# befelix/safe_learning

Measured on NVIDIA B200. Metric: grid-point Lyapunov checks/sec (2D pendulum, M=500 GP), higher is better.
Workload: dtype f64

## Files before the change

### safe_learning_b200/csrc/filter.cu

```cuda
#define SLB_EVAL_NOINLINE 1
#include "common.cuh"

#include <atomic>
#include <string.h>
#include <stdlib.h>

#include "gp_mean_staged.cuh"
#include "gp_args.h"

namespace {

#ifndef SLB_FT
#define SLB_FT 64
#endif
#ifndef SLB_MEAN_MINB
#define SLB_MEAN_MINB 7
#endif
constexpr int FT = SLB_FT;
constexpr int HR = SLB_HEAD_RANK;
constexpr int HT = 512;
constexpr int HEAD_CTAS = 148;
constexpr int64_t CHUNK = 1 << 22;
constexpr int64_t WS_HEAD = 64 + SLB_SPLIT_TICKET_BYTES + (int64_t)SLB_SPLIT_PARTIAL_BYTES;


struct filter_side { double dec0, thr, guard, coef[SLB_MAX_OUT], z[SLB_MAX_IN], dm[SLB_MAX_OUT]; };

struct filter_args {
    int64_t n;
    int64_t idx_begin;
    uint8_t* negative;
    double* values;
    int64_t* list_a;
    filter_side* side_a;
    int64_t* list_b;
    unsigned long long* counts;
    unsigned long long* stats;
    int chunk_rows;
    int max_outputs_per_factor;
    int head_factors_staged;
    int screened;
    int mean_off[SLB_MAX_OUT];
    int mean_doubles;
    int prefetch_factors;
    double* probe_mu;
    double* probe_dm;
};

SLB_DEV int decide(const filter_side& t, const double* shi, int d) {
    double ub = 0.0, lb = 0.0;
    for (int j = 0; j < d; ++j) {
        const double e = t.coef[j] * shi[j];
        ub += fmax(e, 0.0);
        lb += fmin(e, 0.0);
        if (!(e == e)) { ub = e; lb = e; break; }
    }
    const double slack = t.guard + 1e-6 * (fabs(ub) + fabs(lb));
    if (t.dec0 + ub + slack < t.thr) return 1;
    if (t.dec0 + lb - slack >= t.thr) return 0;
    return -1;
}

SLB_DEV long long list_append(bool take, unsigned long long* counter) {
    const unsigned ballot = __ballot_sync(0xffffffffu, take);
    if (ballot == 0) return -1;
    const int lane = threadIdx.x & 31;
    unsigned long long base = 0;
    if (lane == __ffs(ballot) - 1) base = atomicAdd(counter, (unsigned long long)__popc(ballot));
    base = __shfl_sync(0xffffffffu, base, __ffs(ballot) - 1);
    return take ? (long long)(base + __popc(ballot & ((1u << lane) - 1))) : -1;
}

SLB_DEV void count_stat(bool hit, unsigned long long* slot) {
    const unsigned ballot = __ballot_sync(0xffffffffu, hit);
    if (ballot != 0 && (threadIdx.x & 31) == 0) atomicAdd(slot, (unsigned long long)__popc(ballot));
}

SLB_DEV void mean_decision_terms(const slb_sweep& cfg, filter_side& t, double vx, const double* mu,
                                 const double* mean_err) {
    const int D = cfg.gp.num_outputs;
    double vm[1];
    eval_fn_small(cfg.lyapunov, mu, vm);
    t.dec0 = f64sub(vm[0], vx);
    double lvmu = 0.0;
    double lverr = 0.0;
    {
        double lv[SLB_MAX_OUT];
        int nl = 1;
        if (cfg.lipschitz_v.kind != SLB_FN_NONE) nl = eval_fn_small(cfg.lipschitz_v, mu, lv);
        else lv[0] = cfg.lv_const;
        for (int j = 0; j < SLB_MAX_OUT; ++j) {
            const double l = j < D ? (nl == 1 ? lv[0] : lv[j]) : 0.0;
            t.coef[j] = j < D ? l * cfg.gp.outputs[j].beta : 0.0;
            if (j < D) { lvmu += fabs(l * mu[j]); lverr += fabs(l) * mean_err[j]; }
        }
    }
    t.guard = 1e-6 * (fabs(vm[0]) + fabs(vx) + fabs(t.thr) + lvmu) + 4.0 * lverr + 1e-300;
}

SLB_DEV double screening_slack(const slb_sweep& cfg, const double* mu, const double* dm,
                               const double* shi) {
    constexpr int NS = 4;
    const int D = cfg.gp.num_outputs;
    const slb_function& V = cfg.lyapunov;
    const int n = V.in_dim;
    double m[NS], d[NS], bs[NS], P[NS][NS];
#pragma unroll
    for (int i = 0; i < NS; ++i) {
        m[i] = i < n ? mu[i] : 0.0;
        d[i] = i < n ? dm[i] : 0.0;
        bs[i] = i < D ? fabs(cfg.gp.outputs[i].beta) * shi[i] : 0.0;
#pragma unroll
        for (int j = 0; j < NS; ++j) P[i][j] = (i < n && j < n) ? __ldg(V.matrix + i * n + j) : 0.0;
// ... 12 lines not shown
    double dl = 0.0;
    const slb_function& L = cfg.lipschitz_v;
    if (L.kind == SLB_FN_LINEAR) {
        const double sc = (L.flags & SLB_FLAG_SCALE) ? fabs(L.out_scale) : 1.0;
        const int mi = L.in_dim, mo = L.out_dim;
        double row[NS];
#pragma unroll
        for (int o = 0; o < NS; ++o) {
            row[o] = 0.0;
#pragma unroll
            for (int i = 0; i < NS; ++i)
                if (o < mo && i < mi) row[o] += fabs(__ldg(L.matrix + o * mi + i)) * d[i];
        }
        if ((L.flags & SLB_FLAG_NORM1) || mo == 1) {
            dl = sc * (row[0] + row[1] + row[2] + row[3]) * (bs[0] + bs[1] + bs[2] + bs[3]);
        } else {
#pragma unroll
            for (int j = 0; j < NS; ++j) dl += sc * row[j] * bs[j];
        }
    }
    return 1.000001 * (dv + dl);
}

template <int DIN>
__global__ void __launch_bounds__(FT, SLB_MEAN_MINB)
filter_mean_kernel(const __grid_constant__ slb_sweep cfg, const filter_args a) {
    extern __shared__ __align__(16) unsigned char smem_raw[];
    pdl_launch_dependents();
    prefetch_descriptor_operands(cfg);
    mean_pipe P;
    double *tab512, *tab64;
    mean_pipe_setup(P, smem_raw, DIN, a.chunk_rows, a.max_outputs_per_factor, cfg.gp, &tab512, &tab64);
    uint64_t* bar = P.bar;
    if (threadIdx.x == 0) mean_pipe_init(P, tab512);
    mean_pipe_start<DIN>(cfg.gp, P);
    __syncthreads();

    const int64_t rel0 = (int64_t)blockIdx.x * FT + threadIdx.x;
    const bool valid = rel0 < a.n;
    const int64_t rel = valid ? rel0 : a.n - 1;
    const int d = cfg.grid.ndim;
    const int D = cfg.gp.num_outputs;

    filter_side t;
    grid_index_to_state(cfg.grid, a.idx_begin + rel, t.z);
    double vx;
    lyapunov_state_terms(cfg, t.z, a.idx_begin + rel, &vx, &t.thr);
    {
        double u[SLB_MAX_OUT];
        const int m = eval_fn_small(cfg.policy, t.z, u);
        for (int c = 0; c < m; ++c) t.z[d + c] = u[c];
    }
    bool sane = true;
#pragma unroll
    for (int c = 0; c < DIN; ++c) sane &= fabs(t.z[c]) < 1e100;

    slb_bulk::mbar_wait(bar + 2, 0);
    double mu[SLB_MAX_OUT];
    double mean_err[SLB_MAX_OUT];
    gp_mean_staged<DIN, true>(cfg.gp, t.z, mu, mean_err, tab512, tab64, P);

    mean_decision_terms(cfg, t, vx, mu, mean_err);

    double shi[SLB_MAX_OUT];
    for (int j = 0; j < D; ++j) {
        const slb_gp_factor& F = cfg.gp.factors[cfg.gp.outputs[j].factor];
        shi[j] = sqrt(F.kernel.num_prims > 0 ? kernel_expr_diag<DIN>(F.kernel, t.z) : F.variance);
    }
    const int outcome = sane ? decide(t, shi, D) : -1;
    const bool undecided = valid && outcome < 0;
    if (valid) {
        a.negative[rel] = outcome > 0 ? 1 : 0;
        if (a.values != nullptr) a.values[rel] = vx;
    }
    const long long slot = list_append(undecided, a.counts + 0);
    if (undecided) { a.list_a[slot] = rel; a.side_a[slot] = t; }
    if (a.stats != nullptr) {
        count_stat(valid && !undecided, a.stats + 0);
        count_stat(valid, a.stats + 3);
    }
}

template <int DIN>
__global__ void __launch_bounds__(FT, SLB_MEAN_MINB)
filter_mean32_kernel(const __grid_constant__ slb_sweep cfg, const filter_args a) {
    extern __shared__ __align__(16) unsigned char smem_raw[];
    __shared__ double s_cen[SLB_MAX_IN];
    pdl_launch_dependents();
    prefetch_descriptor_operands(cfg);
    constexpr int W32 = row32<DIN>::W;
    mean_pipe P;
    P.bar = reinterpret_cast<uint64_t*>(smem_raw);
    P.C = a.chunk_rows;
    P.xstride = P.C * (DIN + 1);
    P.gstride = P.C * a.max_outputs_per_factor;
    P.xbuf = reinterpret_cast<double*>(smem_raw + 32);
    P.gbuf = P.xbuf + 2 * P.xstride;
    P.t = 0;
    mean32_bufs B;
    B.red = P.gbuf + 2 * P.gstride;
    B.xf = reinterpret_cast<float*>(B.red + 8 * (FT / 32) + 8);
    B.g = B.xf + P.C * W32;
    if (threadIdx.x == 0) {
        slb_bulk::mbar_init(P.bar + 0, 1);
        slb_bulk::mbar_init(P.bar + 1, 1);
        slb_bulk::fence_barrier_init();
        slb_bulk::fence_proxy_async();
    }
    mean_pipe_start<DIN>(cfg.gp, P);

    const int64_t rel0 = (int64_t)blockIdx.x * FT + threadIdx.x;
    const bool valid = rel0 < a.n;
    const int64_t rel = valid ? rel0 : a.n - 1;
    const int d = cfg.grid.ndim;
    const int D = cfg.gp.num_outputs;

    filter_side t;
    grid_index_to_state(cfg.grid, a.idx_begin + rel, t.z);
    double vx;
    lyapunov_state_terms(cfg, t.z, a.idx_begin + rel, &vx, &t.thr);
    {
        double u[SLB_MAX_OUT];
        const int m = eval_fn_small(cfg.policy, t.z, u);
        for (int c = 0; c < m; ++c) t.z[d + c] = u[c];
    }
    bool sane = true;
#pragma unroll
    for (int c = 0; c < DIN; ++c) sane &= fabs(t.z[c]) < 1e100;
    if (threadIdx.x == FT / 2) {
#pragma unroll
        for (int c = 0; c < DIN; ++c) s_cen[c] = t.z[c];
    }
    __syncthreads();
    double zcen[DIN];
#pragma unroll
    for (int c = 0; c < DIN; ++c) zcen[c] = s_cen[c];

    double mu[SLB_MAX_OUT], dm[SLB_MAX_OUT];
    gp_mean32_staged<DIN>(cfg.gp, t.z, zcen, mu, dm, sane, P, B);
    if (a.probe_mu != nullptr && valid) {
        for (int o = 0; o < D; ++o) {
            a.probe_mu[rel * D + o] = mu[o];
            a.probe_dm[rel * D + o] = sane ? dm[o] : __longlong_as_double(0x7ff0000000000000ll);
        }
    }

    double zero[SLB_MAX_OUT];
    for (int j = 0; j < SLB_MAX_OUT; ++j) zero[j] = 0.0;
    mean_decision_terms(cfg, t, vx, mu, zero);
    double shi[SLB_MAX_OUT];
    for (int j = 0; j < D; ++j) shi[j] = sqrt(cfg.gp.factors[cfg.gp.outputs[j].factor].variance);
    t.guard += screening_slack(cfg, mu, dm, shi);
    const int outcome = sane ? decide(t, shi, D) : -1;
    const bool undecided = valid && outcome < 0;
    if (valid) {
        a.negative[rel] = outcome > 0 ? 1 : 0;
        if (a.values != nullptr) a.values[rel] = vx;
    }
    const long long slot = list_append(undecided, a.counts + 0);
    if (undecided) {
        filter_side* dst = a.side_a + slot;
        dst->dec0 = vx;
        dst->thr = t.thr;
#pragma unroll
        for (int c = 0; c < DIN; ++c) dst->z[c] = t.z[c];
        for (int j = 0; j < D; ++j) {
            dst->coef[j] = mu[j];
            dst->dm[j] = sane ? dm[j] : __longlong_as_double(0x7ff0000000000000ll);
        }
        a.list_a[slot] = rel;
    }
    if (a.stats != nullptr) {
        count_stat(valid && !undecided, a.stats + 0);
        count_stat(valid, a.stats + 3);
    }
}

constexpr int HW = HT / 32;
constexpr int HP = 8;
constexpr int HP_SHORT = 2;

template <int DIN, int NO>
SLB_DEV void head_mean_factor(const double* __restrict__ xf, int Mp, const double* zs, double zz, int r,
                              int L, const double* __restrict__ tab512, double* dot) {
    constexpr int W = DIN + 1;
    const double* __restrict__ gm = xf + (size_t)Mp * W;
    double d0[NO], d1[NO];
#pragma unroll
    for (int q = 0; q < NO; ++q) { d0[q] = 0.0; d1[q] = 0.0; }
    for (int j = r; j < Mp; j += 4 * L) {
        double arg[4];
#pragma unroll
        for (int u = 0; u < 4; ++u) {
            const int jc = min(j + L * u, Mp - 1);
            double row[W];
            load_row<W>(xf + jc * W, row);
            double acc = row[DIN] + zz;
#pragma unroll
            for (int c = 0; c < DIN; ++c) acc = fma(zs[c], row[c], acc);
            arg[u] = acc;
        }
#pragma unroll
        for (int u = 0; u < 4; ++u) {
            bool far;
            double k = exp_neg_fast(arg[u], tab512, far);
            k = (far || j + L * u >= Mp) ? 0.0 : k;
            const int jc = min(j + L * u, Mp - 1);
#pragma unroll
            for (int q = 0; q < NO; ++q) {
                if (u & 1) d1[q] = fma(k, gm[q * Mp + jc], d1[q]);
                else d0[q] = fma(k, gm[q * Mp + jc], d0[q]);
            }
        }
    }
#pragma unroll
    for (int q = 0; q < NO; ++q) {
        double v = d0[q] + d1[q];
        for (int off = L >> 1; off > 0; off >>= 1) v += __shfl_xor_sync(0xffffffffu, v, off);
        dot[q] = v;
    }
}

template <int DIN>
SLB_DEV void head_round_means(const slb_sweep& cfg, const filter_args& a, const int* slots, int nneed,
                              int64_t grp0, int64_t count, const double* mbuf, const double* tab512,
                              double* mu_s, double* merr_s) {
    const int nf = cfg.gp.num_factors, D = cfg.gp.num_outputs;
    const int L = nneed <= 16 ? 32 : nneed <= 32 ? 16 : nneed <= 64 ? 8 : 4;
    const int r = threadIdx.x & (L - 1);
    const int per_warp = 32 / L;
    const int nloop = (nneed + per_warp - 1) / per_warp * per_warp;
    for (int i = threadIdx.x / L; i < nloop; i += HT / L) {
        const bool live = i < nneed;
        const int slot = live ? slots[i] : 0;
        const int64_t k = (grp0 + (int64_t)(slot / HP) * gridDim.x) * HP + (slot % HP);
        double z[DIN];
#pragma unroll
        for (int c = 0; c < DIN; ++c) z[c] = (live && k < count) ? a.side_a[k].z[c] : 0.0;
        for (int f = 0; f < nf; ++f) {
            const slb_gp_factor& F = cfg.gp.factors[f];
            int outs[SLB_MAX_OUT];
            int no = 0;
            for (int o = 0; o < D; ++o)
                if (cfg.gp.outputs[o].factor == f) outs[no++] = o;
            double zs[DIN];
            double zz = 0.0;
#pragma unroll
            for (int c = 0; c < DIN; ++c) {
                zs[c] = z[c] / F.lengthscales[c];
                zz = fma(zs[c], zs[c], zz);
            }
            zz *= -0.5;
            const int Mp = padded_rows(F.M);
            const double* xf = mbuf + a.mean_off[f];
            double dot[SLB_MAX_OUT];
            switch (no) {
            case 1: head_mean_factor<DIN, 1>(xf, Mp, zs, zz, r, L, tab512, dot); break;
// ... 261 lines not shown
                if (need) need_s[2 + atomicAdd(need_s + (round & 1), 1)] = warp * HP + lane;
            } else {
                outcome = mine ? decide(t, shi, cfg.gp.num_outputs) : 0;
            }
        }
        if (a.screened) {
            if (threadIdx.x == 0) need_s[(round + 1) & 1] = 0;
            __syncthreads();
            const int nneed = need_s[round & 1];
            if (nneed > 0) {
                head_round_means<DIN>(cfg, a, need_s + 2, nneed, grp0, count, mbuf, tab512, mu_s, merr_s);
                __syncthreads();
                if (need) {
                    double mu[SLB_MAX_OUT], merr[SLB_MAX_OUT];
                    const int slot = warp * HP + lane;
                    for (int j = 0; j < SLB_MAX_OUT; ++j) {
                        mu[j] = mu_s[slot * SLB_MAX_OUT + j];
                        merr[j] = merr_s[slot * SLB_MAX_OUT + j];
                    }
                    mean_decision_terms(cfg, t, vx, mu, merr);
                    outcome = decide(t, shi, cfg.gp.num_outputs);
                }
            }
        }
        if (active) head_group_finish(a, mine, outcome, rel, s_stat);
    }
    __syncthreads();
    if (a.stats != nullptr && threadIdx.x < 2 && s_stat[threadIdx.x] != 0)
        atomicAdd(a.stats + 1 + threadIdx.x, (unsigned long long)s_stat[threadIdx.x]);
}

double* g_probe_mu = nullptr;
double* g_probe_dm = nullptr;
int g_filter_stages = 3;

bool screening_applicable(const slb_sweep& cfg) {
    if (g_filter_stages & 4) return false;
    const int D = cfg.gp.num_outputs;
    for (int f = 0; f < cfg.gp.num_factors; ++f)
        if (cfg.gp.factors[f].kernel.num_prims > 0) return false;
    const slb_function& V = cfg.lyapunov;
    if (D > 4) return false;
    if (V.kind != SLB_FN_QUADRATIC || V.in_dim != D || (V.flags & ~(uint32_t)SLB_FLAG_SCALE)) return false;
    const slb_function& L = cfg.lipschitz_v;
    if (L.kind == SLB_FN_NONE) return true;
    if (L.kind != SLB_FN_LINEAR || L.in_dim != D) return false;
    if (L.flags & ~(uint32_t)(SLB_FLAG_ABS | SLB_FLAG_NORM1 | SLB_FLAG_SCALE)) return false;
    if (L.out_dim > 4) return false;
    return (L.flags & SLB_FLAG_NORM1) || L.out_dim == 1 || L.out_dim == D;
}

void head_layout(const slb_sweep& cfg, int din, filter_args& ah, size_t& head_smem) {
    const size_t head_fixed = 16 + (576 + HW * HR * HP) * sizeof(double);
    const size_t per_factor = (size_t)(HR * HR + HR * din) * sizeof(double);
    ah.head_factors_staged = cfg.gp.num_factors;
    while (ah.head_factors_staged > 0 && head_fixed + ah.head_factors_staged * per_factor > 226 * 1024)
        --ah.head_factors_staged;
    head_smem = head_fixed + ah.head_factors_staged * per_factor;
    ah.screened = 0;
    ah.mean_doubles = 0;
    static const int head_prefetch = [] {
        const char* e = getenv("SLB200_HEAD_PREFETCH");
        return e ? (atoi(e) != 0) : 1;
    }();
    ah.prefetch_factors = ((g_filter_stages & 2) && head_prefetch) ? 1 : 0;
    if (screening_applicable(cfg) && ah.head_factors_staged == cfg.gp.num_factors) {
        int off = 0;
        for (int f = 0; f < cfg.gp.num_factors; ++f) {
            int no = 0;
            for (int o = 0; o < cfg.gp.num_outputs; ++o) no += cfg.gp.outputs[o].factor == f;
            ah.mean_off[f] = off;
            off += ((cfg.gp.factors[f].M + 7) & ~7) * (din + 1 + no);
        }
        const size_t extra = ((size_t)off + 2 * HW * HP * SLB_MAX_OUT) * sizeof(double) +
                             (size_t)(HW * HP + 4) * sizeof(int);
        if (head_smem + extra <= 226 * 1024) {
            ah.screened = 1;
            ah.mean_doubles = off;
            head_smem += extra;
        }
    }
}

template <int DIN>
int launch_filter(cudaStream_t st, const slb_sweep& cfg, const filter_args& a, size_t smem) {
    static std::atomic<bool> configured[64];
    int device = 0;
    SLB_CUDA(cudaGetDevice(&device));
    if (device < 0 || device >= 64 || !configured[device].load(std::memory_order_acquire)) {
        SLB_CUDA(cudaFuncSetAttribute(filter_mean_kernel<DIN>,
                                      cudaFuncAttributeMaxDynamicSharedMemorySize, 96 * 1024));
        SLB_CUDA(cudaFuncSetAttribute(filter_mean32_kernel<DIN>,
                                      cudaFuncAttributeMaxDynamicSharedMemorySize, 96 * 1024));
        SLB_CUDA(cudaFuncSetAttribute(filter_head_kernel<DIN>,
                                      cudaFuncAttributeMaxDynamicSharedMemorySize, 227 * 1024));
        if (device >= 0 && device < 64) configured[device].store(true, std::memory_order_release);
    }
    const int64_t blocks = (a.n + FT - 1) / FT;
    filter_args ah = a;
    size_t head_smem = 0;
    head_layout(cfg, DIN, ah, head_smem);
    ah.probe_mu = g_probe_mu;
    ah.probe_dm = g_probe_dm;
    if (ah.screened) {
        const size_t smem32 = mean32_smem_bytes(DIN, a.max_outputs_per_factor, a.chunk_rows, FT / 32);
        filter_mean32_kernel<DIN><<<(unsigned)blocks, FT, smem32, st>>>(cfg, ah);
    } else {
        filter_mean_kernel<DIN><<<(unsigned)blocks, FT, smem, st>>>(cfg, a);
    }
    SLB_LAUNCH_CHECK();
    if (!(g_filter_stages & 1)) return 0;
    SLB_CUDA(slb_launch_dependent(filter_head_kernel<DIN>, dim3(HEAD_CTAS), dim3(HT), head_smem, st, cfg, ah));
    SLB_LAUNCH_CHECK();
    return 0;
}

}

int slb_launch_refine(cudaStream_t st, const slb_sweep& cfg, int64_t n_max, int64_t idx_begin,
                      const int64_t* list, const unsigned long long* count, uint8_t* negative,
                      double* values, double* split_partial, int* split_ticket);

extern "C" {

int slb_debug_filter_stages(int32_t mask) {
    g_filter_stages = mask;
    return 0;
}

int slb_filter_stage1(const slb_sweep* cfg) {
    if (cfg == nullptr || cfg->gp.num_outputs <= 0) return 0;
    filter_args a;
    memset(&a, 0, sizeof(a));
    size_t smem = 0;
    head_layout(*cfg, cfg->gp.input_dim, a, smem);
    return a.screened ? 32 : 64;
}

int slb_debug_screening_probe(double* mu_dev, double* dm_dev) {
    g_probe_mu = (mu_dev != nullptr && dm_dev != nullptr) ? mu_dev : nullptr;
    g_probe_dm = g_probe_mu != nullptr ? dm_dev : nullptr;
    return 0;
}

int64_t slb_filter_workspace(int64_t n) {
    if (n < 0) n = 0;
    if (n > CHUNK) n = CHUNK;
    return WS_HEAD + n * (int64_t)(2 * sizeof(int64_t) + sizeof(filter_side));
}

int slb_lyapunov_sweep_filtered(void* stream, const slb_sweep* cfg, int64_t idx_begin,
                                int64_t idx_end, uint8_t* negative_dev, double* values_dev,
                                void* workspace_dev, int64_t* stats_dev) {
    SLB_CHECK(cfg != nullptr, "slb_lyapunov_sweep_filtered: null config");
    SLB_CHECK(idx_begin >= 0 && idx_end >= idx_begin && idx_end <= cfg->grid.nindex,
              "slb_lyapunov_sweep_filtered: index range [%lld, %lld) outside the grid (nindex %lld)",
              (long long)idx_begin, (long long)idx_end, (long long)cfg->grid.nindex);
    const int64_t n_all = idx_end - idx_begin;
    if (n_all == 0) return 0;
    SLB_CHECK(negative_dev != nullptr && workspace_dev != nullptr,
              "slb_lyapunov_sweep_filtered: negative_dev and workspace_dev are required");
    if (slb_validate_grid(&cfg->grid, false)) return 1;
    const int d = cfg->grid.ndim;
    if (slb_validate_function(&cfg->policy, "policy", d)) return 1;
    SLB_CHECK(cfg->policy.kind != SLB_FN_NONE, "lyapunov sweep: a policy is required");
    if (slb_validate_function(&cfg->lyapunov, "lyapunov_function", d)) return 1;
    SLB_CHECK(cfg->lyapunov.kind != SLB_FN_NONE, "lyapunov sweep: a Lyapunov function is required");
    if (slb_validate_function(&cfg->lipschitz_v, "lipschitz_lyapunov", d)) return 1;
    if (slb_validate_function(&cfg->lipschitz_f, "lipschitz_dynamics", d)) return 1;
    const int m = (cfg->policy.flags & SLB_FLAG_NORM1) ? 1 : cfg->policy.out_dim;
    SLB_CHECK(m >= 1 && m <= SLB_MAX_ACT, "policy output dim %d unsupported", m);
    SLB_CHECK(cfg->gp.num_outputs > 0, "slb_lyapunov_sweep_filtered needs GP dynamics "
              "(deterministic dynamics have nothing to filter: use slb_lyapunov_sweep)");
    if (slb_validate_gp(&cfg->gp)) return 1;
    SLB_CHECK(cfg->gp.num_outputs == d, "GP stack has %d outputs but the state has %d dims",
              cfg->gp.num_outputs, d);
    SLB_CHECK(cfg->gp.input_dim == d + m, "GP input_dim %d != state %d + action %d",
              cfg->gp.input_dim, d, m);
    int nomax = 1;
    for (int f = 0; f < cfg->gp.num_factors; ++f) {
        const slb_gp_factor& F = cfg->gp.factors[f];
        SLB_CHECK(F.M == 0 || (F.Xf != nullptr && F.Whead != nullptr && F.Wheadp != nullptr &&
                               F.Xhead != nullptr),
                  "filtered sweep: GP factor %d lacks the filter tables (Xf / Whead / Wheadp / Xhead)", f);
        SLB_CHECK(F.M == 0 || ((reinterpret_cast<uintptr_t>(F.Wheadp) & 15) == 0 &&
                               (reinterpret_cast<uintptr_t>(F.Xhead) & 15) == 0),
                  "filtered sweep: GP factor %d: Wheadp / Xhead must be 16-byte aligned", f);
        SLB_CHECK(F.head_rows >= 0 && F.head_rows <= SLB_HEAD_RANK && F.head_rows <= F.M,
                  "filtered sweep: GP factor %d has %d head rows (0..min(M, %d))", f, F.head_rows,
                  SLB_HEAD_RANK);
        SLB_CHECK((reinterpret_cast<uintptr_t>(F.Xf) & 15) == 0,
// ... 61 lines not shown
```

### safe_learning_b200/csrc/gp_mean_staged.cuh

```cuda
#pragma once
#include "common.cuh"
#include "bulk_copy.cuh"
#include "exp2_tab512.cuh"

#ifndef SLB_MEAN_UNROLL
#define SLB_MEAN_UNROLL 4
#endif
constexpr int MEAN_UNROLL = SLB_MEAN_UNROLL;
constexpr double EPS_K = 1.0e-13;

SLB_DEV double exp_neg_fast(double x, const double* __restrict__ tab, bool& far) {
    const double MAGIC = 6755399441055744.0;
    const double t = fma(x, 738.6598609351493, MAGIC);
    const int n = __double2loint(t);
    const double nd = t - MAGIC;
    const double r = fma(nd, -0.0013538030870311431, x);
    double q = fma(r, 1.0 / 6.0, 0.5);
    q = q * r;
    const double p = fma(q, r, r);
    const double T = tab[n & 511];
    const double v = fma(T, p, T);
    far = (unsigned)__double2hiint(x) > 0xC085E000u;
    return __hiloint2double(__double2hiint(v) + ((n >> 9) << 20), __double2loint(v));
}
// ... 163 lines not shown
}

template <int DIN>
SLB_DEV void mean_pipe_start(const slb_gp_stack& gp, mean_pipe& P) {
    P.pf = first_factor_with_data(gp, 0);
    P.pc0 = 0;
    if (threadIdx.x == 0) issue_slice<DIN>(gp, P, P.t & 1);
}

template <int DIN, bool FAST>
SLB_DEV void gp_mean_staged(const slb_gp_stack& gp, const double* z, double* mu, double* mean_err,
                            const double* tab512, const double* tab64, mean_pipe& P) {
    for (int f = 0; f < gp.num_factors; ++f) {
        int outs[SLB_MAX_OUT];
        int no = 0;
        for (int o = 0; o < gp.num_outputs; ++o)
            if (gp.outputs[o].factor == f) outs[no++] = o;
        switch (no) {
        case 1: mean_factor<DIN, 1, FAST>(gp, f, outs, z, mu, mean_err, tab512, tab64, P); break;
        case 2: mean_factor<DIN, 2, FAST>(gp, f, outs, z, mu, mean_err, tab512, tab64, P); break;
        case 3: mean_factor<DIN, 3, FAST>(gp, f, outs, z, mu, mean_err, tab512, tab64, P); break;
        case 4: mean_factor<DIN, 4, FAST>(gp, f, outs, z, mu, mean_err, tab512, tab64, P); break;
        case 5: mean_factor<DIN, 5, FAST>(gp, f, outs, z, mu, mean_err, tab512, tab64, P); break;
        case 6: mean_factor<DIN, 6, FAST>(gp, f, outs, z, mu, mean_err, tab512, tab64, P); break;
        default: break;
        }
    }
}

SLB_DEV void mean_pipe_setup(mean_pipe& P, unsigned char* smem_raw, int din, int chunk_rows, int nomax,
                             const slb_gp_stack& gp, double** tab512, double** tab64) {
    P.bar = reinterpret_cast<uint64_t*>(smem_raw);
    *tab512 = reinterpret_cast<double*>(smem_raw + 32);
    *tab64 = *tab512 + 512;
    P.C = chunk_rows;
    P.xstride = P.C * (din + 1);
    P.gstride = P.C * nomax;
    P.xbuf = *tab64 + 64;
    P.gbuf = P.xbuf + 2 * P.xstride;
    P.t = 0;
    P.pf = first_factor_with_data(gp, 0);
    P.pc0 = 0;
}

inline int mean_chunk_rows(int din, int nomax, int budget_kb) {
    const int rows = (budget_kb * 1024) / (2 * 8 * (din + 1 + nomax));
    return rows >= 256 ? 256 : (rows & ~7);
}
inline size_t mean_smem_bytes(int din, int nomax, int chunk_rows) {
    return 32 + (512 + 64) * sizeof(double) + (size_t)2 * chunk_rows * (din + 1 + nomax) * sizeof(double);
}

constexpr int F32_FLUSH = 16;

template <int DIN>
struct row32 { static constexpr int W = DIN + 1 <= 2 ? 2 : (DIN + 1 <= 4 ? 4 : 8); };

SLB_DEV float ex2_approx(float x) {
    float y;
    asm("ex2.approx.ftz.f32 %0, %1;" : "=f"(y) : "f"(x));
    return y;
}

template <int W32>
SLB_DEV void load_row32(const float* __restrict__ p, float (&r)[W32]) {
    if constexpr (W32 == 2) {
        const float2 v = *reinterpret_cast<const float2*>(p);
        r[0] = v.x; r[1] = v.y;
    } else {
#pragma unroll
        for (int c = 0; c < W32; c += 4) {
            const float4 v = *reinterpret_cast<const float4*>(p + c);
            r[c] = v.x; r[c + 1] = v.y; r[c + 2] = v.z; r[c + 3] = v.w;
        }
    }
}

struct mean32_bufs {
    float* xf;
    float* g;
    double* red;
};

template <int DIN, int NO>
SLB_DEV void mean32_factor(const slb_gp_stack& gp, int f, const int* outs, const double* z,
                           const double* zcen, double* mu, double* dmu, bool& ok, mean_pipe& P,
                           const mean32_bufs& B) {
    const slb_gp_factor& F = gp.factors[f];
    constexpr int W = DIN + 1, W32 = row32<DIN>::W;
    const double S = 1.2011224087864498;
    __syncthreads();
    if (threadIdx.x < DIN) {
        B.red[threadIdx.x] = zcen[threadIdx.x] / F.lengthscales[threadIdx.x];
        B.red[DIN + threadIdx.x] = S / F.lengthscales[threadIdx.x];
    }
    __syncthreads();
    double cs[DIN];
    float zc[DIN];
    double Z = 0.0;
#pragma unroll
    for (int c = 0; c < DIN; ++c) {
        cs[c] = B.red[c];
        const double zcd = (z[c] - zcen[c]) * B.red[DIN + c];
        zc[c] = (float)zcd;
        Z = fma(zcd, zcd, Z);
        if (!(fabs(cs[c]) < 1e4) || !(fabs(zcd) < 1e4)) ok = false;
    }
    Z *= 0.5;
    __syncthreads();
    float acc[NO][4];
    double dot[NO], g1[NO];
#pragma unroll
    for (int q = 0; q < NO; ++q) {
        dot[q] = 0.0; g1[q] = 0.0;
#pragma unroll
        for (int u = 0; u < 4; ++u) acc[q][u] = 0.0f;
    }
    const int Mp = padded_rows(F.M);
    for (int c0 = 0; c0 < Mp; c0 += P.C) {
        const int rows = min(P.C, Mp - c0);
        const int b = P.t & 1;
        if (threadIdx.x == 0) issue_slice<DIN>(gp, P, b ^ 1);
        slb_bulk::mbar_wait(P.bar + b, (P.t >> 1) & 1);
        const double* __restrict__ xb = P.xbuf + b * P.xstride;
        const double* __restrict__ gb = P.gbuf + b * P.gstride;
        for (int r = threadIdx.x; r < rows; r += blockDim.x) {
            double row[W];
            load_row<W>(xb + r * W, row);
            float o[W32];
            double hh = 0.0;
#pragma unroll
            for (int c = 0; c < DIN; ++c) {
                const double xcd = (row[c] - cs[c]) * S;
                o[c] = (float)xcd;
                hh = fma(xcd, xcd, hh);
            }
            o[DIN] = (float)(-0.5 * hh);
#pragma unroll
            for (int c = DIN + 1; c < W32; ++c) o[c] = 0.0f;
            float* dst = B.xf + r * W32;
            if constexpr (W32 == 2) {
                *reinterpret_cast<float2*>(dst) = make_float2(o[0], o[1]);
            } else {
#pragma unroll
                for (int c = 0; c < W32; c += 4)
                    *reinterpret_cast<float4*>(dst + c) = make_float4(o[c], o[c + 1], o[c + 2], o[c + 3]);
            }
#pragma unroll
            for (int q = 0; q < NO; ++q) {
                const double gq = gb[q * P.C + r];
                B.g[q * P.C + r] = (float)gq;
                g1[q] += fabs(gq);
            }
        }
        __syncthreads();
        const float* __restrict__ xf = B.xf;
        const float* __restrict__ gf = B.g;
        for (int jb = 0; jb < rows; jb += 4 * F32_FLUSH) {
            const int jend = min(jb + 4 * F32_FLUSH, rows);
            for (int j0 = jb; j0 < jend; j0 += 4) {
                float k[4];
#pragma unroll
                for (int u = 0; u < 4; ++u) {
                    float row[W32];
                    load_row32<W32>(xf + (j0 + u) * W32, row);
                    float arg = row[DIN];
#pragma unroll
                    for (int c = 0; c < DIN; ++c) arg = fmaf(zc[c], row[c], arg);
                    k[u] = ex2_approx(arg);
                }
#pragma unroll
                for (int q = 0; q < NO; ++q) {
                    const float4 g = *reinterpret_cast<const float4*>(gf + q * P.C + j0);
                    acc[q][0] = fmaf(k[0], g.x, acc[q][0]);
                    acc[q][1] = fmaf(k[1], g.y, acc[q][1]);
                    acc[q][2] = fmaf(k[2], g.z, acc[q][2]);
                    acc[q][3] = fmaf(k[3], g.w, acc[q][3]);
                }
            }
#pragma unroll
            for (int q = 0; q < NO; ++q) {
                dot[q] += ((double)acc[q][0] + (double)acc[q][1]) + ((double)acc[q][2] + (double)acc[q][3]);
#pragma unroll
                for (int u = 0; u < 4; ++u) acc[q][u] = 0.0f;
            }
        }
        __syncthreads();
        ++P.t;
    }
    const int lane = threadIdx.x & 31, warp = threadIdx.x >> 5, nw = (blockDim.x + 31) >> 5;
#pragma unroll
    for (int q = 0; q < NO; ++q) {
        double v = g1[q];
#pragma unroll
        for (int off = 16; off > 0; off >>= 1) v += __shfl_xor_sync(0xffffffffu, v, off);
        if (lane == 0) B.red[q * nw + warp] = v;
    }
    __syncthreads();
    const double E = (double)ex2_approx(-(float)Z);
    const double u24 = 5.9604644775390625e-8;
    const double epsrel = u24 * (0.7 * (DIN + 2.01) * (2.13 + 5.0 * Z) + 11.0 + F32_FLUSH + 8.0 + 0.7 * Z);
    if (!(Z <= 40.0)) ok = false;
#pragma unroll
    for (int q = 0; q < NO; ++q) {
        double gsum = 0.0;
        for (int w = 0; w < nw; ++w) gsum += B.red[q * nw + w];
        const slb_gp_output& G = gp.outputs[outs[q]];
        double mx = 0.0;
        if (G.prior_mean != nullptr) {
            mx = f64mul(z[0], G.prior_mean[0]);
#pragma unroll
            for (int c = 1; c < DIN; ++c) mx = f64add(mx, f64mul(z[c], G.prior_mean[c]));
            mx = f64mul(F.scale, mx);
        }
        mu[outs[q]] = f64add(E * dot[q], mx) / F.scale;
        dmu[outs[q]] = (1.05 * epsrel * gsum + 1.3e-26 * Mp) / fabs(F.scale) + 1e-300;
    }
}

template <int DIN>
SLB_DEV void gp_mean32_staged(const slb_gp_stack& gp, const double* z, const double* zcen, double* mu,
                              double* dmu, bool& ok, mean_pipe& P, const mean32_bufs& B) {
    for (int f = 0; f < gp.num_factors; ++f) {
        int outs[SLB_MAX_OUT];
        int no = 0;
        for (int o = 0; o < gp.num_outputs; ++o)
            if (gp.outputs[o].factor == f) outs[no++] = o;
        switch (no) {
        case 1: mean32_factor<DIN, 1>(gp, f, outs, z, zcen, mu, dmu, ok, P, B); break;
        case 2: mean32_factor<DIN, 2>(gp, f, outs, z, zcen, mu, dmu, ok, P, B); break;
        case 3: mean32_factor<DIN, 3>(gp, f, outs, z, zcen, mu, dmu, ok, P, B); break;
        case 4: mean32_factor<DIN, 4>(gp, f, outs, z, zcen, mu, dmu, ok, P, B); break;
        case 5: mean32_factor<DIN, 5>(gp, f, outs, z, zcen, mu, dmu, ok, P, B); break;
        case 6: mean32_factor<DIN, 6>(gp, f, outs, z, zcen, mu, dmu, ok, P, B); break;
        default: break;
        }
    }
}

inline size_t mean32_smem_bytes(int din, int nomax, int chunk_rows, int warps) {
    const int w32 = din + 1 <= 2 ? 2 : (din + 1 <= 4 ? 4 : 8);
    return 32 + (size_t)2 * chunk_rows * (din + 1 + nomax) * sizeof(double) +
           (size_t)chunk_rows * (w32 + nomax) * sizeof(float) + (size_t)(8 * warps + 8) * sizeof(double);
}
```

Measured before the change: 436.7 million.

## Screen grid points in 2D tiles with multi-point-per-thread GP mean

The screening mean kernel now maps each CTA to a 2D tile of the last two grid dimensions (8x16 by default, 128 threads) instead of a contiguous run of 64 flat indices. The tile center serves as the expansion point, so the float32 centered arguments stay small and more points pass the screen without a fallback. The GP mean routine is templated on points per thread so that each loaded training row can be reused across several query points, though the default is one point per thread. The change also adds index mapping overhead, partial tiles at chunk boundaries, and a lower min-blocks launch bound.

```diff
diff --git a/safe_learning_b200/csrc/filter.cu b/safe_learning_b200/csrc/filter.cu
--- a/safe_learning_b200/csrc/filter.cu
+++ b/safe_learning_b200/csrc/filter.cu
@@ -17,6 +17,21 @@
 #define SLB_MEAN_MINB 7
 #endif
 constexpr int FT = SLB_FT;
+#ifndef SLB_TILE_R
+#define SLB_TILE_R 8
+#endif
+#ifndef SLB_TILE_C
+#define SLB_TILE_C 16
+#endif
+#ifndef SLB_PPT
+#define SLB_PPT 1
+#endif
+#ifndef SLB_MEAN32_MINB
+#define SLB_MEAN32_MINB 4
+#endif
+constexpr int TILE_R = SLB_TILE_R, TILE_C = SLB_TILE_C, PPT = SLB_PPT;
+constexpr int FT32 = TILE_R * TILE_C / PPT;
+static_assert(FT32 % 32 == 0 && FT32 * PPT == TILE_R * TILE_C, "screening tile: whole warps per CTA");
 constexpr int HR = SLB_HEAD_RANK;
 constexpr int HT = 512;
 constexpr int HEAD_CTAS = 148;
@@ -26,9 +41,12 @@
 
 struct filter_side { double dec0, thr, guard, coef[SLB_MAX_OUT], z[SLB_MAX_IN], dm[SLB_MAX_OUT]; };
 
+struct screen_tiles { int64_t nrow, ncol, row_tiles, col_tiles, g0; int tr, tc; };
+
 struct filter_args {
     int64_t n;
     int64_t idx_begin;
+    screen_tiles tiles;
     uint8_t* negative;
     double* values;
     int64_t* list_a;
@@ -207,11 +225,33 @@
 }
 
 template <int DIN>
-__global__ void __launch_bounds__(FT, SLB_MEAN_MINB)
+__global__ void __launch_bounds__(FT32, SLB_MEAN32_MINB)
 filter_mean32_kernel(const __grid_constant__ slb_sweep cfg, const filter_args a) {
     extern __shared__ __align__(16) unsigned char smem_raw[];
     __shared__ double s_cen[SLB_MAX_IN];
     pdl_launch_dependents();
+    const screen_tiles& T = a.tiles;
+    const int64_t g = T.g0 + blockIdx.x / T.col_tiles;
+    const int64_t plane = g / T.row_tiles;
+    const int64_t row0 = (g % T.row_tiles) * T.tr, col0 = (blockIdx.x % T.col_tiles) * T.tc;
+    const int64_t base = plane * T.nrow;
+    const int64_t flat_c = min(((base + min(row0 + T.tr / 2, T.nrow - 1)) * T.ncol +
+                                min(col0 + T.tc / 2, T.ncol - 1)), cfg.grid.nindex - 1);
+    const int pmid = (T.tr / 2) * T.tc + T.tc / 2;
+    int64_t idx[PPT];
+    bool valid[PPT];
+#pragma unroll
+    for (int k = 0; k < PPT; ++k) {
+        const int p = threadIdx.x + k * FT32;
+        const int64_t row = row0 + p / T.tc, col = col0 + p % T.tc;
+        const int64_t flat = (base + row) * T.ncol + col;
+        valid[k] = row < T.nrow && col < T.ncol && flat >= a.idx_begin && flat < a.idx_begin + a.n;
+        idx[k] = valid[k] ? flat : flat_c;
+    }
+    bool any = false;
+#pragma unroll
+    for (int k = 0; k < PPT; ++k) any |= valid[k];
+    if (!__syncthreads_or(any)) return;
     prefetch_descriptor_operands(cfg);
     constexpr int W32 = row32<DIN>::W;
     mean_pipe P;
@@ -224,7 +264,7 @@
     P.t = 0;
     mean32_bufs B;
     B.red = P.gbuf + 2 * P.gstride;
-    B.xf = reinterpret_cast<float*>(B.red + 8 * (FT / 32) + 8);
+    B.xf = reinterpret_cast<float*>(B.red + 8 * (FT32 / 32) + 8);
     B.g = B.xf + P.C * W32;
     if (threadIdx.x == 0) {
         slb_bulk::mbar_init(P.bar + 0, 1);
@@ -234,70 +274,83 @@
     }
     mean_pipe_start<DIN>(cfg.gp, P);
 
-    const int64_t rel0 = (int64_t)blockIdx.x * FT + threadIdx.x;
-    const bool valid = rel0 < a.n;
-    const int64_t rel = valid ? rel0 : a.n - 1;
     const int d = cfg.grid.ndim;
     const int D = cfg.gp.num_outputs;
 
-    filter_side t;
-    grid_index_to_state(cfg.grid, a.idx_begin + rel, t.z);
-    double vx;
-    lyapunov_state_terms(cfg, t.z, a.idx_begin + rel, &vx, &t.thr);
-    {
+    filter_side t[PPT];
+    double vx[PPT];
+    bool sane[PPT];
+#pragma unroll
+    for (int k = 0; k < PPT; ++k) grid_index_to_state(cfg.grid, idx[k], t[k].z);
+#pragma unroll
+    for (int k = 0; k < PPT; ++k)
+        lyapunov_state_terms(cfg, t[k].z, valid[k] ? idx[k] : -1, &vx[k], &t[k].thr);
+#pragma unroll
+    for (int k = 0; k < PPT; ++k) {
         double u[SLB_MAX_OUT];
-        const int m = eval_fn_small(cfg.policy, t.z, u);
-        for (int c = 0; c < m; ++c) t.z[d + c] = u[c];
-    }
-    bool sane = true;
-#pragma unroll
-    for (int c = 0; c < DIN; ++c) sane &= fabs(t.z[c]) < 1e100;
-    if (threadIdx.x == FT / 2) {
-#pragma unroll
-        for (int c = 0; c < DIN; ++c) s_cen[c] = t.z[c];
+        const int m = eval_fn_small(cfg.policy, t[k].z, u);
+        for (int c = 0; c < m; ++c) t[k].z[d + c] = u[c];
+        sane[k] = true;
+#pragma unroll
+        for (int c = 0; c < DIN; ++c) sane[k] &= fabs(t[k].z[c]) < 1e100;
+        if (threadIdx.x + k * FT32 == pmid) {
+#pragma unroll
+            for (int c = 0; c < DIN; ++c) s_cen[c] = t[k].z[c];
+        }
     }
     __syncthreads();
     double zcen[DIN];
 #pragma unroll
     for (int c = 0; c < DIN; ++c) zcen[c] = s_cen[c];
 
-    double mu[SLB_MAX_OUT], dm[SLB_MAX_OUT];
-    gp_mean32_staged<DIN>(cfg.gp, t.z, zcen, mu, dm, sane, P, B);
-    if (a.probe_mu != nullptr && valid) {
-        for (int o = 0; o < D; ++o) {
-            a.probe_mu[rel * D + o] = mu[o];
-            a.probe_dm[rel * D + o] = sane ? dm[o] : __longlong_as_double(0x7ff0000000000000ll);
-        }
-    }
-
+    double mu[PPT][SLB_MAX_OUT], dm[PPT][SLB_MAX_OUT];
+    const double* zp[PPT];
+#pragma unroll
+    for (int k = 0; k < PPT; ++k) zp[k] = t[k].z;
+    gp_mean32_staged<DIN, PPT>(cfg.gp, zp, zcen, mu, dm, sane, P, B);
+
+    double shi[SLB_MAX_OUT];
+    for (int j = 0; j < D; ++j) shi[j] = sqrt(cfg.gp.factors[cfg.gp.outputs[j].factor].variance);
     double zero[SLB_MAX_OUT];
     for (int j = 0; j < SLB_MAX_OUT; ++j) zero[j] = 0.0;
-    mean_decision_terms(cfg, t, vx, mu, zero);
-    double shi[SLB_MAX_OUT];
-    for (int j = 0; j < D; ++j) shi[j] = sqrt(cfg.gp.factors[cfg.gp.outputs[j].factor].variance);
-    t.guard += screening_slack(cfg, mu, dm, shi);
-    const int outcome = sane ? decide(t, shi, D) : -1;
-    const bool undecided = valid && outcome < 0;
-    if (valid) {
-        a.negative[rel] = outcome > 0 ? 1 : 0;
-        if (a.values != nullptr) a.values[rel] = vx;
-    }
-    const long long slot = list_append(undecided, a.counts + 0);
-    if (undecided) {
-        filter_side* dst = a.side_a + slot;
-        dst->dec0 = vx;
-        dst->thr = t.thr;
-#pragma unroll
-        for (int c = 0; c < DIN; ++c) dst->z[c] = t.z[c];
-        for (int j = 0; j < D; ++j) {
-            dst->coef[j] = mu[j];
-            dst->dm[j] = sane ? dm[j] : __longlong_as_double(0x7ff0000000000000ll);
-        }
-        a.list_a[slot] = rel;
-    }
-    if (a.stats != nullptr) {
-        count_stat(valid && !undecided, a.stats + 0);
-        count_stat(valid, a.stats + 3);
+    int outcome[PPT];
+#pragma unroll
+    for (int k = 0; k < PPT; ++k) {
+        mean_decision_terms(cfg, t[k], vx[k], mu[k], zero);
+        t[k].guard += screening_slack(cfg, mu[k], dm[k], shi);
+        outcome[k] = sane[k] ? decide(t[k], shi, D) : -1;
+    }
+#pragma unroll
+    for (int k = 0; k < PPT; ++k) {
+        const int64_t rel = idx[k] - a.idx_begin;
+        if (a.probe_mu != nullptr && valid[k]) {
+            for (int o = 0; o < D; ++o) {
+                a.probe_mu[rel * D + o] = mu[k][o];
+                a.probe_dm[rel * D + o] = sane[k] ? dm[k][o] : __longlong_as_double(0x7ff0000000000000ll);
+            }
+        }
+        const bool undecided = valid[k] && outcome[k] < 0;
+        if (valid[k]) {
+            a.negative[rel] = outcome[k] > 0 ? 1 : 0;
+            if (a.values != nullptr) a.values[rel] = vx[k];
+        }
+        const long long slot = list_append(undecided, a.counts + 0);
+        if (undecided) {
+            filter_side* dst = a.side_a + slot;
+            dst->dec0 = vx[k];
+            dst->thr = t[k].thr;
+#pragma unroll
+            for (int c = 0; c < DIN; ++c) dst->z[c] = t[k].z[c];
+            for (int j = 0; j < D; ++j) {
+                dst->coef[j] = mu[k][j];
+                dst->dm[j] = sane[k] ? dm[k][j] : __longlong_as_double(0x7ff0000000000000ll);
+            }
+            a.list_a[slot] = rel;
+        }
+        if (a.stats != nullptr) {
+            count_stat(valid[k] && !undecided, a.stats + 0);
+            count_stat(valid[k], a.stats + 3);
+        }
     }
 }
 
@@ -725,6 +778,28 @@
     }
 }
 
+int64_t screen_tiles_plan(const slb_grid& g, int64_t idx_begin, int64_t n, screen_tiles& T) {
+    if (g.ndim >= 2) {
+        T.nrow = g.num_points[g.ndim - 2];
+        T.ncol = g.num_points[g.ndim - 1];
+        T.tr = TILE_R;
+        T.tc = TILE_C;
+    } else {
+        T.tc = TILE_R * TILE_C;
+        T.tr = 1;
+        T.ncol = T.tc;
+        T.nrow = (g.nindex + T.tc - 1) / T.tc;
+    }
+    T.row_tiles = (T.nrow + T.tr - 1) / T.tr;
+    T.col_tiles = (T.ncol + T.tc - 1) / T.tc;
+    auto row_tile = [&](int64_t i) {
+        const int64_t r = i / T.ncol;
+        return (r / T.nrow) * T.row_tiles + (r % T.nrow) / T.tr;
+    };
+    T.g0 = row_tile(idx_begin);
+    return (row_tile(idx_begin + n - 1) - T.g0 + 1) * T.col_tiles;
+}
+
 template <int DIN>
 int launch_filter(cudaStream_t st, const slb_sweep& cfg, const filter_args& a, size_t smem) {
     static std::atomic<bool> configured[64];
@@ -739,17 +814,17 @@
                                       cudaFuncAttributeMaxDynamicSharedMemorySize, 227 * 1024));
         if (device >= 0 && device < 64) configured[device].store(true, std::memory_order_release);
     }
-    const int64_t blocks = (a.n + FT - 1) / FT;
     filter_args ah = a;
     size_t head_smem = 0;
     head_layout(cfg, DIN, ah, head_smem);
     ah.probe_mu = g_probe_mu;
     ah.probe_dm = g_probe_dm;
     if (ah.screened) {
-        const size_t smem32 = mean32_smem_bytes(DIN, a.max_outputs_per_factor, a.chunk_rows, FT / 32);
-        filter_mean32_kernel<DIN><<<(unsigned)blocks, FT, smem32, st>>>(cfg, ah);
+        const int64_t blocks = screen_tiles_plan(cfg.grid, a.idx_begin, a.n, ah.tiles);
+        const size_t smem32 = mean32_smem_bytes(DIN, a.max_outputs_per_factor, a.chunk_rows, FT32 / 32);
+        filter_mean32_kernel<DIN><<<(unsigned)blocks, FT32, smem32, st>>>(cfg, ah);
     } else {
-        filter_mean_kernel<DIN><<<(unsigned)blocks, FT, smem, st>>>(cfg, a);
+        filter_mean_kernel<DIN><<<(unsigned)((a.n + FT - 1) / FT), FT, smem, st>>>(cfg, a);
     }
     SLB_LAUNCH_CHECK();
     if (!(g_filter_stages & 1)) return 0;
diff --git a/safe_learning_b200/csrc/gp_mean_staged.cuh b/safe_learning_b200/csrc/gp_mean_staged.cuh
--- a/safe_learning_b200/csrc/gp_mean_staged.cuh
+++ b/safe_learning_b200/csrc/gp_mean_staged.cuh
@@ -269,10 +269,10 @@
     double* red;
 };
 
-template <int DIN, int NO>
-SLB_DEV void mean32_factor(const slb_gp_stack& gp, int f, const int* outs, const double* z,
-                           const double* zcen, double* mu, double* dmu, bool& ok, mean_pipe& P,
-                           const mean32_bufs& B) {
+template <int DIN, int NO, int NP>
+SLB_DEV void mean32_factor(const slb_gp_stack& gp, int f, const int* outs, const double* const* z,
+                           const double* zcen, double (*mu)[SLB_MAX_OUT], double (*dmu)[SLB_MAX_OUT],
+                           bool* ok, mean_pipe& P, const mean32_bufs& B) {
     const slb_gp_factor& F = gp.factors[f];
     constexpr int W = DIN + 1, W32 = row32<DIN>::W;
     const double S = 1.2011224087864498;
@@ -283,25 +283,34 @@
     }
     __syncthreads();
     double cs[DIN];
-    float zc[DIN];
-    double Z = 0.0;
-#pragma unroll
-    for (int c = 0; c < DIN; ++c) {
-        cs[c] = B.red[c];
-        const double zcd = (z[c] - zcen[c]) * B.red[DIN + c];
-        zc[c] = (float)zcd;
-        Z = fma(zcd, zcd, Z);
-        if (!(fabs(cs[c]) < 1e4) || !(fabs(zcd) < 1e4)) ok = false;
-    }
-    Z *= 0.5;
+    float zc[NP][DIN];
+    double Z[NP];
+#pragma unroll
+    for (int c = 0; c < DIN; ++c) cs[c] = B.red[c];
+#pragma unroll
+    for (int p = 0; p < NP; ++p) {
+        Z[p] = 0.0;
+#pragma unroll
+        for (int c = 0; c < DIN; ++c) {
+            const double zcd = (z[p][c] - zcen[c]) * B.red[DIN + c];
+            zc[p][c] = (float)zcd;
+            Z[p] = fma(zcd, zcd, Z[p]);
+            if (!(fabs(cs[c]) < 1e4) || !(fabs(zcd) < 1e4)) ok[p] = false;
+        }
+        Z[p] *= 0.5;
+    }
     __syncthreads();
-    float acc[NO][4];
-    double dot[NO], g1[NO];
+    float acc[NP][NO][4];
+    double dot[NP][NO], g1[NO];
 #pragma unroll
     for (int q = 0; q < NO; ++q) {
-        dot[q] = 0.0; g1[q] = 0.0;
-#pragma unroll
-        for (int u = 0; u < 4; ++u) acc[q][u] = 0.0f;
+        g1[q] = 0.0;
+#pragma unroll
+        for (int p = 0; p < NP; ++p) {
+            dot[p][q] = 0.0;
+#pragma unroll
+            for (int u = 0; u < 4; ++u) acc[p][q][u] = 0.0f;
+        }
     }
     const int Mp = padded_rows(F.M);
     for (int c0 = 0; c0 < Mp; c0 += P.C) {
@@ -346,31 +355,40 @@
         for (int jb = 0; jb < rows; jb += 4 * F32_FLUSH) {
             const int jend = min(jb + 4 * F32_FLUSH, rows);
             for (int j0 = jb; j0 < jend; j0 += 4) {
-                float k[4];
+                float k[NP][4];
 #pragma unroll
                 for (int u = 0; u < 4; ++u) {
                     float row[W32];
                     load_row32<W32>(xf + (j0 + u) * W32, row);
-                    float arg = row[DIN];
-#pragma unroll
-                    for (int c = 0; c < DIN; ++c) arg = fmaf(zc[c], row[c], arg);
-                    k[u] = ex2_approx(arg);
+#pragma unroll
+                    for (int p = 0; p < NP; ++p) {
+                        float arg = row[DIN];
+#pragma unroll
+                        for (int c = 0; c < DIN; ++c) arg = fmaf(zc[p][c], row[c], arg);
+                        k[p][u] = ex2_approx(arg);
+                    }
                 }
 #pragma unroll
                 for (int q = 0; q < NO; ++q) {
                     const float4 g = *reinterpret_cast<const float4*>(gf + q * P.C + j0);
-                    acc[q][0] = fmaf(k[0], g.x, acc[q][0]);
-                    acc[q][1] = fmaf(k[1], g.y, acc[q][1]);
-                    acc[q][2] = fmaf(k[2], g.z, acc[q][2]);
-                    acc[q][3] = fmaf(k[3], g.w, acc[q][3]);
-                }
-            }
-#pragma unroll
-            for (int q = 0; q < NO; ++q) {
-                dot[q] += ((double)acc[q][0] + (double)acc[q][1]) + ((double)acc[q][2] + (double)acc[q][3]);
-#pragma unroll
-                for (int u = 0; u < 4; ++u) acc[q][u] = 0.0f;
-            }
+#pragma unroll
+                    for (int p = 0; p < NP; ++p) {
+                        acc[p][q][0] = fmaf(k[p][0], g.x, acc[p][q][0]);
+                        acc[p][q][1] = fmaf(k[p][1], g.y, acc[p][q][1]);
+                        acc[p][q][2] = fmaf(k[p][2], g.z, acc[p][q][2]);
+                        acc[p][q][3] = fmaf(k[p][3], g.w, acc[p][q][3]);
+                    }
+                }
+            }
+#pragma unroll
+            for (int p = 0; p < NP; ++p)
+#pragma unroll
+                for (int q = 0; q < NO; ++q) {
+                    dot[p][q] += ((double)acc[p][q][0] + (double)acc[p][q][1]) +
+                                 ((double)acc[p][q][2] + (double)acc[p][q][3]);
+#pragma unroll
+                    for (int u = 0; u < 4; ++u) acc[p][q][u] = 0.0f;
+                }
         }
         __syncthreads();
         ++P.t;
@@ -384,42 +402,50 @@
         if (lane == 0) B.red[q * nw + warp] = v;
     }
     __syncthreads();
-    const double E = (double)ex2_approx(-(float)Z);
     const double u24 = 5.9604644775390625e-8;
-    const double epsrel = u24 * (0.7 * (DIN + 2.01) * (2.13 + 5.0 * Z) + 11.0 + F32_FLUSH + 8.0 + 0.7 * Z);
-    if (!(Z <= 40.0)) ok = false;
+    double gsum[NO];
 #pragma unroll
     for (int q = 0; q < NO; ++q) {
-        double gsum = 0.0;
-        for (int w = 0; w < nw; ++w) gsum += B.red[q * nw + w];
-        const slb_gp_output& G = gp.outputs[outs[q]];
-        double mx = 0.0;
-        if (G.prior_mean != nullptr) {
-            mx = f64mul(z[0], G.prior_mean[0]);
-#pragma unroll
-            for (int c = 1; c < DIN; ++c) mx = f64add(mx, f64mul(z[c], G.prior_mean[c]));
-            mx = f64mul(F.scale, mx);
-        }
-        mu[outs[q]] = f64add(E * dot[q], mx) / F.scale;
-        dmu[outs[q]] = (1.05 * epsrel * gsum + 1.3e-26 * Mp) / fabs(F.scale) + 1e-300;
-    }
-}
-
-template <int DIN>
-SLB_DEV void gp_mean32_staged(const slb_gp_stack& gp, const double* z, const double* zcen, double* mu,
-                              double* dmu, bool& ok, mean_pipe& P, const mean32_bufs& B) {
+        gsum[q] = 0.0;
+        for (int w = 0; w < nw; ++w) gsum[q] += B.red[q * nw + w];
+    }
+#pragma unroll
+    for (int p = 0; p < NP; ++p) {
+        const double E = (double)ex2_approx(-(float)Z[p]);
+        const double epsrel = u24 * (0.7 * (DIN + 2.01) * (2.13 + 5.0 * Z[p]) + 11.0 + F32_FLUSH + 8.0 + 0.7 * Z[p]);
+        if (!(Z[p] <= 40.0)) ok[p] = false;
+#pragma unroll
+        for (int q = 0; q < NO; ++q) {
+            const slb_gp_output& G = gp.outputs[outs[q]];
+            double mx = 0.0;
+            if (G.prior_mean != nullptr) {
+                mx = f64mul(z[p][0], G.prior_mean[0]);
+#pragma unroll
+                for (int c = 1; c < DIN; ++c) mx = f64add(mx, f64mul(z[p][c], G.prior_mean[c]));
+                mx = f64mul(F.scale, mx);
+            }
+            mu[p][outs[q]] = f64add(E * dot[p][q], mx) / F.scale;
+            dmu[p][outs[q]] = (1.05 * epsrel * gsum[q] + 1.3e-26 * Mp) / fabs(F.scale) + 1e-300;
+        }
+    }
+}
+
+template <int DIN, int NP>
+SLB_DEV void gp_mean32_staged(const slb_gp_stack& gp, const double* const* z, const double* zcen,
+                              double (*mu)[SLB_MAX_OUT], double (*dmu)[SLB_MAX_OUT], bool* ok,
+                              mean_pipe& P, const mean32_bufs& B) {
     for (int f = 0; f < gp.num_factors; ++f) {
         int outs[SLB_MAX_OUT];
         int no = 0;
         for (int o = 0; o < gp.num_outputs; ++o)
             if (gp.outputs[o].factor == f) outs[no++] = o;
         switch (no) {
-        case 1: mean32_factor<DIN, 1>(gp, f, outs, z, zcen, mu, dmu, ok, P, B); break;
-        case 2: mean32_factor<DIN, 2>(gp, f, outs, z, zcen, mu, dmu, ok, P, B); break;
-        case 3: mean32_factor<DIN, 3>(gp, f, outs, z, zcen, mu, dmu, ok, P, B); break;
-        case 4: mean32_factor<DIN, 4>(gp, f, outs, z, zcen, mu, dmu, ok, P, B); break;
-        case 5: mean32_factor<DIN, 5>(gp, f, outs, z, zcen, mu, dmu, ok, P, B); break;
-        case 6: mean32_factor<DIN, 6>(gp, f, outs, z, zcen, mu, dmu, ok, P, B); break;
+        case 1: mean32_factor<DIN, 1, NP>(gp, f, outs, z, zcen, mu, dmu, ok, P, B); break;
+        case 2: mean32_factor<DIN, 2, NP>(gp, f, outs, z, zcen, mu, dmu, ok, P, B); break;
+        case 3: mean32_factor<DIN, 3, NP>(gp, f, outs, z, zcen, mu, dmu, ok, P, B); break;
+        case 4: mean32_factor<DIN, 4, NP>(gp, f, outs, z, zcen, mu, dmu, ok, P, B); break;
+        case 5: mean32_factor<DIN, 5, NP>(gp, f, outs, z, zcen, mu, dmu, ok, P, B); break;
+        case 6: mean32_factor<DIN, 6, NP>(gp, f, outs, z, zcen, mu, dmu, ok, P, B); break;
         default: break;
         }
     }
```

New measurement: 439.8 million, median of 6. About the same (+0.7%).
